# NomaDamas/AutoRAG-Research

Hardware: AMD Instinct MI355X
Metric: queries/sec (higher is better)
Workload: dtype f32

## Files before the change

autorag_research_amd/csrc/index.h:

```cpp
#pragma once
#include <climits>
#include <hip/hip_runtime.h>

#include <algorithm>
#include <cmath>
#include <cstdio>
#include <cstring>
#include <mutex>
#include <string>
#include <vector>

#include "dev_common.h"
#include "mi355dr.h"

namespace mi355 {
struct EventPair {
    hipEvent_t a, b;
    int big;
};
struct MultiVecStore;
struct Pending {
    bool active = false;
    hipEvent_t done = nullptr;
    int* status_host = nullptr;
// ... 30 lines not shown
    mi355::I8Group* grp8 = nullptr;
    int32_t* irr8_rows = nullptr;
    int* irr8_count = nullptr;
    int irr8_n = 0;

    bool qstate_ready = false;
    mi355::QueryState st{};
    float* qdev = nullptr;
    int32_t* cand_row = nullptr;
    float* cand_val = nullptr;
    int* qlist_dev = nullptr;
    int* status_or_dev = nullptr;
    int* status_host = nullptr;
    double* out_dist_dev = nullptr;
    int64_t* out_rows_dev = nullptr;
    unsigned long long* stat_dev = nullptr;
    int* prune_skip = nullptr;
    int prune_parity = 0;

    int path = 0;
    int screen_dtype = 0;
    int retry_level = 0;
    int i8_backoff = 0, i8_probation = 0;
    int i8_demoted_k = INT_MAX;
    double i8_min_budget = 0.25;
    float* retry_q[3] = {nullptr, nullptr, nullptr};
    double* retry_dist[3] = {nullptr, nullptr, nullptr};
    int64_t* retry_rows[3] = {nullptr, nullptr, nullptr};
    int* retry_map[3] = {nullptr, nullptr, nullptr};
    mi355::Pending pend[mi355::kPendingRing];
    mi355::Pending sub_pend[4];
    int64_t seq_next = 0, seq_done = 0;
    int k_now = 10;
    bool screening_now = false;
    int maxsim_coop = -1;
    int maxsim_persistent = 0;
    int maxsim_wg = -1;
    int maxsim_tighten = 1;
    int maxsim_aligned = 1;
    int maxsim_wg_min = 8;
    int maxsim_wg_pipe = 1;
    int maxsim_pack8 = -1;
    int maxsim_wg_bps = 4;
    int maxsim_pass_groups = 4;
    int maxsim_screen = 1;
    int64_t row_offset = 0;
    int round_a = 0;
    int screen_rq = 1;
    int screen_stream = 1;
    int prefilter16 = 0;
    int profile = 0;
    int starter = 1;
    int prune_companion = 1;
    int scan_dma = 1;
    int defer_round_b = 1;
    int chunk0_set = 0;
    int64_t chunk0_rows = 1024;
    int64_t chunk_growth = 3;
    int chunk_growth_set = 0;
    int64_t small_chunk_rows = 16384;
    int cap = mi355::kCandCap;
    int cap_set = 0;
    int prune_wide = 1;
    int screen_flush_sync = 1, screen_flush_lanes = 48, screen_flush_alone = 40;
    int wide_inflation_x10 = 100;
    int flush_mask_now = -1;
    int chunk_taper_x100 = 0;
    int64_t starter_rows_wide = 65536;

    int64_t s_screen_launches = 0, s_screen_ns = 0, s_screen_rows = 0, s_fallback_queries = 0, s_chunks = 0,
            s_passes = 0, s_candidates = 0, s_rescored = 0, s_starters = 0;
    int64_t s_big_launches = 0, s_big_ns = 0, s_big_rows = 0;
    int screen_rq_split_tests = 1;
    int64_t debug_park = 0;
    float* park_thr = nullptr;
    int screen_drift = 3;
    int* rq_progress = nullptr;
    int rq_epoch = 0;
    int64_t s_rq_launches = 0;
    int64_t s_retry_queries = 0;
    int64_t s_ms_screened = 0, s_ms_candidates = 0, s_ms_fallbacks = 0;
    int64_t s_ms_screen_ns = 0, s_ms_screen_launches = 0, s_ms_exact_ns = 0, s_ms_exact_launches = 0, s_ms_pack_ns = 0;
    int64_t s_ms_packed_launches = 0;
    int64_t s_ms_packed_blocks = 0;
    int64_t s_ms_packed_built = 0;
    int64_t s_ms_screen_cols = 0;
    hipEvent_t ms_ev[4] = {nullptr, nullptr, nullptr, nullptr};
    std::vector<mi355::EventPair> ev_pool, ev_pending;
    hipEvent_t t0 = nullptr, t1 = nullptr;

    void* comm = nullptr;
    int comm_rank = 0, comm_world = 0;
    mi355dr_allgather_fn comm_custom = nullptr;
    void* comm_custom_user = nullptr;
    int64_t* comm_packed[2] = {nullptr, nullptr};
    int64_t* comm_packed_all[2] = {nullptr, nullptr};
    hipStream_t comm_stream = nullptr;
    hipEvent_t comm_done[2] = {nullptr, nullptr};
    bool comm_done_armed[2] = {false, false};
    size_t comm_cap = 0;

    mi355::MultiVecStore* mv = nullptr;
};


namespace mi355 {
// ... 35 lines not shown
```

autorag_research_amd/csrc/k_select.h:

```cpp
#pragma once
#include "dev_common.h"

namespace mi355 {

struct PruneArgs {
    const float* rows;
    const float* nrm2;
    const float* q;
    QueryState st;
    int32_t* cand_row;
    float* cand_val;
    const int* qlist;
    unsigned long long* stat;
    int cap, d, k, metric;
    int exact;
    const uint8_t* flag8;
    float cscale;
    const uint16_t* shadow16;
    int dpad;
    int round_a;
    int* skip_list;
    int skip_parity;
    int thr_only;
    int one_wave_only;
    int defer_b;
};

__device__ __forceinline__ float unit_sim(int metric, double dist, float inv_qn) {
    return metric == 0 ? (float)(1.0 - dist) : (float)(-dist) * inv_qn;
}
__device__ __forceinline__ float screen_threshold(int metric, double dist_k, float E, float nq) {
    if (metric == 0) return float_below((float)((1.0 - dist_k) - (double)E));
    const double u = -dist_k / sqrt((double)nq);
    return float_below((float)(u - fabs(u) * 4e-6 - (double)E));
}

constexpr int kPruneSmallThreads = 64, kPruneSmallSort = 1024;
constexpr int kPruneBigThreads = 256, kPruneBigSort = kSortMax;

__host__ __device__ inline size_t prune_qs_floats(int d) { return ((size_t)d + 3) / 4 * 4 + 16; }
__host__ __device__ inline size_t prune_lds_bytes(int d, int threads, int sortmax, int dpad16) {
    size_t x = (size_t)(threads / kWave) * kStageFloats * sizeof(float);
    size_t lf = (size_t)sortmax * sizeof(float);
    if (lf > x) x = lf;
    return (size_t)sortmax * 8 + (size_t)sortmax * 4 + x + (size_t)sortmax * 4 + prune_qs_floats(d) * 4 + (size_t)dpad16 * 4;
}

template <int PER, int T, bool ROWS = false>
__device__ __forceinline__ void load_candidate_keys(uint32_t (&key)[PER], const float* __restrict__ cval,
                                                    const int32_t* __restrict__ crow, const uint8_t* __restrict__ flag8,
                                                    int n_new, int tid, int32_t* rows_out = nullptr) {
    float v[PER];
    int32_t r[PER];
    const int last = n_new - 1;
#pragma unroll
    for (int j = 0; j < PER; ++j) {
        v[j] = 0.0f;
        r[j] = 0;
        if (j * T >= n_new) continue;
        v[j] = cval[min(j * T + tid, last)];
        if (ROWS) r[j] = crow[min(j * T + tid, last)];
    }
    uint8_t f[PER];
#pragma unroll
    for (int j = 0; j < PER; ++j) f[j] = 0;
    if (flag8 != nullptr) {
        if (!ROWS) {
#pragma unroll
            for (int j = 0; j < PER; ++j) {
                if (j * T >= n_new) continue;
                r[j] = crow[min(j * T + tid, last)];
            }
        }
#pragma unroll
        for (int j = 0; j < PER; ++j) {
            if (j * T >= n_new) continue;
            f[j] = flag8[r[j]];
        }
    }
// ... 3 lines not shown
        if (j * T + tid < n_new) {
            if (v[j] != v[j]) kk = 0xFFFFFFFFu;
            else if (!f[j]) kk = f32_order_key(v[j]);
        }
        key[j] = kk;
        if (ROWS) rows_out[j] = r[j];
    }
}

template <int THREADS, int SORT>
__device__ __forceinline__ void prune_body(const PruneArgs& a, char* smem);

template <int THREADS, int SORT>
__global__ __launch_bounds__(THREADS) void k_prune(PruneArgs a) {
    extern __shared__ __attribute__((aligned(16))) char smem[];
    const bool list_mode = a.skip_list != nullptr && a.qlist == nullptr;
    const int tid = threadIdx.x;
    const int lane = tid & 63, wave = tid >> 6;
    int q = a.qlist ? a.qlist[blockIdx.x] : blockIdx.x;
    if (SORT == kPruneBigSort && list_mode) {
        if (blockIdx.x == 0 && tid == 0) a.skip_list[a.skip_parity ^ 1] = 0;
        const int n_left = a.skip_list[a.skip_parity];
        for (int i = blockIdx.x; i < n_left; i += gridDim.x) {
            PruneArgs b = a;
            b.skip_list = nullptr;
            b.qlist = a.skip_list + 2 + a.skip_parity * kQBlockMax + i - 0;
            b.qlist -= blockIdx.x;
            prune_body<THREADS, SORT>(b, smem);
            __syncthreads();
        }
        return;
    }
    prune_body<THREADS, SORT>(a, smem);
}

template <int THREADS, int SORT>
__device__ __forceinline__ void prune_body(const PruneArgs& a, char* smem) {
    constexpr int kWaves = THREADS / kWave;
    uint64_t* SK = (uint64_t*)smem;
    int32_t* SR = (int32_t*)(smem + (size_t)SORT * 8);
    char* X = smem + (size_t)SORT * 12;
    constexpr size_t xa = (size_t)kWaves * kStageFloats * sizeof(float), xb = (size_t)SORT * sizeof(float);
    constexpr size_t xbytes = xa > xb ? xa : xb;
    float* Lf = (float*)X;
    float* tiles = (float*)X;
    int32_t* R = (int32_t*)(X + xbytes);
    float* qs = (float*)(X + xbytes + (size_t)SORT * 4);
    int& s_cnt = *(int*)(X + xbytes + (size_t)SORT * 4 + (prune_qs_floats(a.d) - 16) * 4);
    float* q16 = qs + prune_qs_floats(a.d);
    const bool list_mode = a.skip_list != nullptr && a.qlist == nullptr;
    const int q = a.qlist ? a.qlist[blockIdx.x] : blockIdx.x;
    const int tid = threadIdx.x;
    const int lane = tid & 63, wave = tid >> 6;
    const int raw_cnt = a.st.cnt[q];
    const int n_best = a.st.best_n[q];
    if (raw_cnt == 0) return;
    if (a.exact && SORT < kPruneBigSort) return;
    auto leave_for_general = [&]() {
        if (a.one_wave_only) {
            if (tid == 0) {
                a.st.status[q] |= kStOverflow;
                a.st.cnt[q] = 0;
            }
            return;
        }
        if (list_mode && tid == 0) {
            const int i = atomicAdd(&a.skip_list[a.skip_parity], 1);
            a.skip_list[2 + a.skip_parity * kQBlockMax + i] = q;
        }
    };
    if (raw_cnt > a.cap) {
        if (SORT < kPruneBigSort) {
            leave_for_general();
            return;
        }
        if (tid == 0) {
            a.st.status[q] |= kStOverflow;
            a.st.cnt[q] = 0;
        }
        return;
    }
    if (n_best + raw_cnt > SORT) {
        if (SORT < kPruneBigSort) {
            leave_for_general();
            return;
        }
        if (tid == 0) {
            a.st.status[q] |= kStOverflow;
            a.st.cnt[q] = 0;
        }
        return;
    }
    const int n_new = raw_cnt;
    const int32_t* crow = a.cand_row + (int64_t)q * a.cap;
    const float* cval = a.cand_val + (int64_t)q * a.cap;
    uint64_t* bkey = a.st.best_key + (int64_t)q * kKMax;
    int32_t* brow = a.st.best_row + (int64_t)q * kKMax;
    const float nq = a.st.qn[q];
    const float inv_qn = 1.0f / sqrtf(nq);
    const float E = a.st.E[q];
    if (tid == 0) {
        a.stat[2 * q] += (unsigned long long)(n_new - a.st.carry[q]);
        a.st.carry[q] = 0;
    }

    int n_res;
    int n_base = n_best;
    bool kept_loaded = false;
    if constexpr (THREADS == kWave) {
        if (!a.exact) {
            float* tile = tiles;
            uint32_t key[kSelPerLane];
            unsigned in_a = 0;
            load_candidate_keys<kSelPerLane, kWave>(key, cval, crow, a.flag8, n_new, lane);
            for (int k = lane; k < a.d; k += kWave) qs[k] = a.q[(int64_t)q * a.d + k];
            if (a.shadow16 != nullptr)
                for (int k = lane; k < a.dpad; k += kWave) q16[k] = bf16_bits_to_f32(a.st.qhat[(int64_t)q * a.dpad + k]);
            const int n_cand = wave_count_ge(key, 1u, n_new);
            auto rescore_list = [&](int n, int dst) __attribute__((always_inline)) {
                for (int base = 0; base < n; base += kWave) {
                    const int e = base + lane;
                    const bool live = e < n;
                    const int32_t row = live ? crow[R[e]] : -1;
                    const float* rp = live ? a.rows + (int64_t)row * a.d : nullptr;
                    const float acc = staged_dot(tile, rp, qs, a.d, lane);
                    if (live) {
                        SK[dst + e] = dist_to_key(distance_from(a.metric, acc, nq, a.nrm2[row]));
                        SR[dst + e] = row;
                    }
                }
            };
            auto compact = [&](uint32_t x, int room, bool mark) -> int {
                int n = 0;
#pragma unroll
                for (int j = 0; j < kSelPerLane; ++j) {
                    if (j * kWave >= n_new) break;
                    const bool want = key[j] >= x && key[j] != 0 && !((in_a >> j) & 1u);
                    const unsigned long long bal = __builtin_amdgcn_ballot_w64(want);
                    const int pos = n + (int)__builtin_amdgcn_mbcnt_hi((unsigned)(bal >> 32),
                                                                       __builtin_amdgcn_mbcnt_lo((unsigned)bal, 0));
                    if (want && pos < room) {
                        R[pos] = j * kWave + lane;
                        if (mark) in_a |= 1u << j;
// ... 103 lines not shown
                    const int e = j * kWave + lane;
                    uint32_t kk = 0;
                    if (e < n_tot) kk = SK[e] == kKeyNaN ? 1u : f32_order_key(sim_of_dist(a.metric, key_to_dist(SK[e])));
                    sk[j] = kk;
                }
                const uint32_t xs = wave_nth_largest(sk, a.k, n_tot);
                n_sel = 0;
#pragma unroll
                for (int j = 0; j < kSelPerLane; ++j) {
                    if (j * kWave >= n_tot) break;
                    const bool want = sk[j] >= xs && sk[j] != 0;
                    const unsigned long long bal = __builtin_amdgcn_ballot_w64(want);
                    const int pos = n_sel + (int)__builtin_amdgcn_mbcnt_hi((unsigned)(bal >> 32),
                                                                           __builtin_amdgcn_mbcnt_lo((unsigned)bal, 0));
                    if (want) {
                        K2[pos] = SK[j * kWave + lane];
                        R2[pos] = SR[j * kWave + lane];
                    }
                    n_sel += __builtin_popcountll(bal);
                }
            } else {
                for (int i = lane; i < n_tot; i += kWave) {
                    K2[i] = SK[i];
                    R2[i] = SR[i];
                }
            }
            const int np = next_pow2(max(n_sel, 1));
            for (int i = n_sel + lane; i < np; i += kWave) {
                K2[i] = kKeyNaN;
                R2[i] = 0x7FFFFFFF;
            }
            __syncthreads();
            bitonic_asc_key_row(K2, R2, np);
            const int n_keep = min(a.k, n_sel);
            if (!a.thr_only)
                for (int i = lane; i < n_keep; i += kWave) {
                    bkey[i] = K2[i];
                    brow[i] = R2[i];
                }
            if (lane == 0) {
                if (!a.thr_only) a.st.best_n[q] = n_keep;
                a.st.cnt[q] = carried;
                a.st.carry[q] = carried;
                if (n_keep >= a.k) {
                    const uint64_t wk = K2[a.k - 1];
                    if (!a.thr_only) {
                        a.st.thr_key[q] = wk;
                        a.st.thr_row[q] = R2[a.k - 1];
                    }
                    if (wk != kKeyNaN && !(a.st.status[q] & kStIrregular))
                        a.st.thr[q] = screen_threshold(a.metric, key_to_dist(wk), E, nq);
                }
            }
            return;
        }
    }
    if (!a.exact) {
        const int nLp = next_pow2(n_new);
        for (int i = tid; i < nLp; i += THREADS) {
            float v = -__builtin_inff();
            if (i < n_new) {
                v = cval[i];
                if (v != v) v = __builtin_inff();
                else if (a.flag8 && a.flag8[crow[i]]) v = -__builtin_inff();
            }
            Lf[i] = v;
            R[i] = i;
        }
        if (tid == 0) s_cnt = 0;
        __syncthreads();
        bitonic_desc_f32_i32(Lf, R, nLp);
        for (int i = tid; i < nLp; i += THREADS)
            if (Lf[i] > -__builtin_inff() && (i + 1 == nLp || !(Lf[i + 1] > -__builtin_inff()))) s_cnt = i + 1;
        for (int k = tid; k < a.d; k += THREADS) qs[k] = a.q[(int64_t)q * a.d + k];
        __syncthreads();
        const int n_cand = s_cnt;
        __syncthreads();
        float* tile = tiles + wave * kStageFloats;
        auto rescore = [&](int e0, int e1, int dst) {
            for (int base = e0; base < e1; base += THREADS) {
                const int e = base + wave * kWave + lane;
                const bool live = e < e1;
                const int32_t row = live ? crow[R[e]] : -1;
                const float* rp = live ? a.rows + (int64_t)row * a.d : nullptr;
                float acc = 0.0f;
                if (base + wave * kWave < e1) acc = staged_dot(tile, rp, qs, a.d, lane);
                if (live) {
                    const double dist = distance_from(a.metric, acc, nq, a.nrm2[row]);
                    SK[dst + (e - e0)] = dist_to_key(dist);
                    SR[dst + (e - e0)] = row;
                }
            }
        };
        const int nA = min(n_cand, min(THREADS, max(32, 2 * a.k)));
        rescore(0, nA, n_best);
        int n_pass = nA;
        if (n_cand > nA) {
            for (int i = tid; i < n_best; i += THREADS) {
                SK[i] = bkey[i];
                SR[i] = brow[i];
            }
            kept_loaded = true;
            const int n1 = n_best + nA;
            const int np1 = next_pow2(n1);
            for (int i = n1 + tid; i < np1; i += THREADS) {
                SK[i] = kKeyNaN;
// ... 12 lines not shown
            }
            if (tid == 0) s_cnt = nA;
            __syncthreads();
            for (int i = nA + tid; i < n_cand; i += THREADS) {
                const float v = cval[R[i]];
                if (!(v < cut)) atomicMax(&s_cnt, i + 1);
            }
            __syncthreads();
            n_pass = s_cnt;
            rescore(nA, n_pass, n_base);
            n_res = n_pass - nA;
        } else {
            n_res = nA;
        }
        if (tid == 0) a.stat[2 * q + 1] += (unsigned long long)n_pass;
    } else {
        n_res = n_new;
        for (int i = tid; i < n_new; i += THREADS) {
            const int32_t row = crow[i];
            const double dist = distance_from(a.metric, cval[i], nq, a.nrm2[row]);
            SK[n_best + i] = dist_to_key(dist);
            SR[n_best + i] = row;
        }
    }
    if (!kept_loaded)
        for (int i = tid; i < n_best; i += THREADS) {
            SK[i] = bkey[i];
            SR[i] = brow[i];
        }
    const int n_tot = n_base + n_res;
    const int np = next_pow2(n_tot);
    for (int i = n_tot + tid; i < np; i += THREADS) {
        SK[i] = kKeyNaN;
        SR[i] = 0x7FFFFFFF;
    }
    __syncthreads();
    bitonic_asc_key_row(SK, SR, np);
    const int n_keep = min(a.k, n_tot);
    for (int i = tid; i < n_keep; i += THREADS) {
        bkey[i] = SK[i];
        brow[i] = SR[i];
    }
    if (tid == 0) {
        a.st.best_n[q] = n_keep;
        a.st.cnt[q] = 0;
        if (n_keep >= a.k) {
            const uint64_t wk = SK[a.k - 1];
            a.st.thr_key[q] = wk;
            a.st.thr_row[q] = SR[a.k - 1];
            if (!a.exact && wk != kKeyNaN && !(a.st.status[q] & kStIrregular))
                a.st.thr[q] = screen_threshold(a.metric, key_to_dist(wk), E, nq);
        }
    }
}

__global__ __launch_bounds__(64) void k_emit_irregular(const int32_t* __restrict__ irr_rows, int irr_n, QueryState st,
                                                        int32_t* cand_row, float* cand_val, int cap, int skip_below) {
    const int q = blockIdx.x;
    if (st.status[q] & kStIrregular) return;
    for (int i = threadIdx.x; i < irr_n; i += blockDim.x) {
        if (irr_rows[i] < skip_below) continue;
        const int slot = atomicAdd(&st.cnt[q], 1);
        if (slot < cap) {
            cand_row[(int64_t)q * cap + slot] = irr_rows[i];
            cand_val[(int64_t)q * cap + slot] = __builtin_nanf("");
        }
    }
}

__global__ __launch_bounds__(64) void k_finalize(QueryState st, int k, int64_t row_offset, double* out_dist,
                                                  int64_t* out_rows, int* status_or) {
    const int q = blockIdx.x;
    const int n = st.best_n[q];
    for (int s = threadIdx.x; s < k; s += blockDim.x) {
        if (s < n) {
            out_dist[(int64_t)q * k + s] = key_to_dist(st.best_key[(int64_t)q * kKMax + s]);
            out_rows[(int64_t)q * k + s] = (int64_t)st.best_row[(int64_t)q * kKMax + s] + row_offset;
        } else {
            out_dist[(int64_t)q * k + s] = __longlong_as_double(0x7FF8000000000000ll);
            out_rows[(int64_t)q * k + s] = -1;
        }
    }
    if (threadIdx.x == 0 && st.status[q] != 0) atomicOr(status_or, st.status[q]);
}

__global__ __launch_bounds__(256) void k_merge_topk(const double* __restrict__ dist_all,
                                                     const int64_t* __restrict__ rows_all, int64_t rank_stride, int world,
                                                     int B, int k, double* out_dist, int64_t* out_rows) {
    extern __shared__ __attribute__((aligned(16))) char smem[];
    uint64_t* SK = (uint64_t*)smem;
    const int np_ = next_pow2(world * k);
    int32_t* SI = (int32_t*)(smem + (size_t)np_ * 8);
    const int q = blockIdx.x;
    const int n = world * k;
    const int np = next_pow2(n);
    for (int i = threadIdx.x; i < np; i += blockDim.x) {
        if (i < n) {
            const int w = i / k, s = i % k;
            const int64_t src = (int64_t)w * rank_stride + (int64_t)q * k + s;
            const int64_t r = rows_all[src];
            SK[i] = r < 0 ? kKeyNaN : dist_to_key(dist_all[src]);
            SI[i] = r < 0 ? 0x7FFFFFFF : i;
        } else {
            SK[i] = kKeyNaN;
            SI[i] = 0x7FFFFFFF;
        }
// ... 51 lines not shown
```

autorag_research_amd/csrc/mi355dr.hip:

```cpp
#include "index.h"
#include "k_prep.h"
#include "k_scan.h"
#include "k_screen.h"
#include "k_screen256c.h"
#include "k_screen_rq.h"

#define MI355_RQ_FORMS(X) X(1) X(2) X(3) X(4) X(5) X(6)
inline bool screen_rq_has(int ksteps) { return ksteps >= 1 && ksteps <= 6; }
#include "k_screen_stream.h"
#include "k_select.h"
#include "k_prune_wide.h"

using namespace mi355;

namespace {
std::mutex g_err_mu;
std::string g_err;
}

namespace mi355 {
int fail(mi355dr_index* idx, int code, const std::string& msg) {
    if (idx) idx->err = msg;
    else {
        std::lock_guard<std::mutex> g(g_err_mu);
// ... 142 lines not shown

EventPair take_events(mi355dr_index* idx) {
    if (!idx->ev_pool.empty()) {
        EventPair p = idx->ev_pool.back();
        idx->ev_pool.pop_back();
        return p;
    }
    EventPair p{};
    (void)hipEventCreate(&p.a);
    (void)hipEventCreate(&p.b);
    return p;
}

void drain_events(mi355dr_index* idx) {
    std::vector<EventPair> keep;
    for (auto& p : idx->ev_pending) {
        if (hipEventQuery(p.b) == hipErrorNotReady) {
            keep.push_back(p);
            continue;
        }
        float ms = 0.f;
        if (hipEventElapsedTime(&ms, p.a, p.b) == hipSuccess) {
            idx->s_screen_ns += (int64_t)(ms * 1e6);
            if (p.big) idx->s_big_ns += (int64_t)(ms * 1e6);
        }
        idx->ev_pool.push_back(p);
    }
    idx->ev_pending.swap(keep);
}

constexpr double kInflationBf16 = 5.0, kInflationI8 = 16.0;
constexpr double kSmallBlockBudget = 1.6;
constexpr double kInflationI8Wide = 10.0, kInflationBf16Wide = 4.0;
inline bool wide_ok(const mi355dr_index* idx, int k) { return idx->prune_wide && k >= kWideKMin && k <= kWideKMax; }
inline bool wide_now(const mi355dr_index* idx) { return idx->screening_now && wide_ok(idx, idx->k_now); }
inline int cap_now(const mi355dr_index* idx) { return !idx->cap_set && wide_now(idx) ? kCandCapWide : idx->cap; }
inline double growth_budget(const mi355dr_index* idx, int k, bool i8) {
    if (wide_ok(idx, k) && idx->path != MI355DR_PATH_SCAN) {
        const int room = std::min(kWideEntries, idx->cap_set ? idx->cap : kCandCapWide);
        return 0.75 * room / ((double)k * (i8 ? idx->wide_inflation_x10 / 10.0 : kInflationBf16Wide)) - 1.0;
    }
    const int room = k < kPruneSmallSort / 2 ? kPruneSmallSort - k : idx->cap;
    return 0.6 * std::min(room, idx->cap) / ((double)k * (i8 ? kInflationI8 : kInflationBf16));
}

inline bool i8_available(const mi355dr_index* idx) { return idx->irr8_n <= kIrrCap; }
inline bool use_i8(const mi355dr_index* idx) {
    if (idx->retry_level > 0) return false;
    if (idx->screen_dtype == MI355DR_SCREEN_I8) return true;
    return idx->screen_dtype == MI355DR_SCREEN_AUTO && i8_available(idx) && idx->k_now < idx->i8_demoted_k &&
           growth_budget(idx, idx->k_now, true) >= idx->i8_min_budget;
}

int launch_prune(mi355dr_index* idx, hipStream_t s, int nblocks, const int* qlist, int k, int exact, bool thr_only = false,
                 bool one_wave_only = false, bool defer_b = false) {
    PruneArgs pa{};
    pa.thr_only = thr_only ? 1 : 0;
    pa.one_wave_only = one_wave_only ? 1 : 0;
    pa.defer_b = defer_b && idx->defer_round_b ? 1 : 0;
    pa.rows = idx->rows;
    pa.nrm2 = idx->nrm2;
    pa.q = idx->qdev;
    pa.st = idx->st;
    pa.cand_row = idx->cand_row;
    pa.cand_val = idx->cand_val;
    pa.qlist = qlist;
    pa.stat = idx->stat_dev;
    pa.cap = cap_now(idx);
    pa.d = idx->dim;
    pa.k = k;
    pa.metric = idx->metric;
    pa.exact = exact;
    pa.flag8 = (use_i8(idx) && idx->irr8_n > 0) ? idx->flag8 : nullptr;
    pa.cscale = idx->metric == MI355DR_METRIC_IP ? idx->cmax : 1.0f;
    pa.shadow16 = (use_i8(idx) && idx->metric == 0 && !exact && idx->prefilter16) ? idx->shadow : nullptr;
    pa.dpad = idx->dpad;
    pa.round_a = idx->round_a;
    if (!exact && wide_now(idx)) {
        pa.shadow16 = nullptr;
        hipLaunchKernelGGL((k_prune_wide<2, 32>), dim3(nblocks), dim3(2 * kWave), prune_wide_lds_bytes(idx->dim, 2), s, pa);
        HIPCHECK(idx, hipGetLastError());
        return MI355DR_OK;
    }
    if (pa.cap > kCandCap) return fail(idx, MI355DR_E_INTERNAL, "general-form prune on a list stride above kCandCap");
    const bool list_mode = qlist == nullptr;
    pa.skip_list = list_mode ? idx->prune_skip : nullptr;
    pa.skip_parity = list_mode ? (idx->prune_parity ^= 1) : 0;
    hipLaunchKernelGGL((k_prune<kPruneSmallThreads, kPruneSmallSort>), dim3(nblocks), dim3(kPruneSmallThreads),
                       prune_lds_bytes(idx->dim, kPruneSmallThreads, kPruneSmallSort, pa.shadow16 ? idx->dpad : 0), s, pa);
    HIPCHECK(idx, hipGetLastError());
    if (one_wave_only) return MI355DR_OK;
    hipLaunchKernelGGL((k_prune<kPruneBigThreads, kPruneBigSort>), dim3(list_mode ? std::min(nblocks, 64) : nblocks),
                       dim3(kPruneBigThreads), prune_lds_bytes(idx->dim, kPruneBigThreads, kPruneBigSort, 0), s, pa);
    HIPCHECK(idx, hipGetLastError());
    return MI355DR_OK;
}

int launch_prep(mi355dr_index* idx, hipStream_t s, int B, int Bpad, int metric, int cnt0 = 0) {
    hipLaunchKernelGGL(k_prep_queries, dim3(Bpad), dim3(64), (size_t)idx->dim * sizeof(float), s, idx->qdev, B, idx->dim,
                       idx->dpad, metric, idx->st, idx->dpad8, use_i8(idx) ? 1 : 0, idx->bf16_ec, idx->status_or_dev,
                       idx->prune_skip, cnt0, idx->metric == MI355DR_METRIC_IP ? idx->cmax : 1.0f);
    idx->prune_parity = 0;
    HIPCHECK(idx, hipGetLastError());
    return MI355DR_OK;
}

inline int screen_tile(int B) { return B > kTileN ? kT2 : kTileM; }

constexpr int kRetryLevels = 2;

__global__ void k_set_counts(int* cnt, int n, int v) {
    const int i = blockIdx.x * blockDim.x + threadIdx.x;
    if (i < n) cnt[i] = v;
}

int launch_screen(mi355dr_index* idx, hipStream_t s, int B, int64_t r0, int64_t r_end, int cap, int emit_mode) {
    const bool emit_all = emit_mode != 0;
    const int tile = (emit_all || r_end - r0 <= idx->small_chunk_rows) ? kTileM : screen_tile(B);
    const bool i8 = use_i8(idx);
    ScreenArgs2 sa{};
    sa.status = idx->st.status;
    sa.shadow = i8 ? (const void*)idx->shadow8 : (const void*)idx->shadow;
    sa.qhat = i8 ? (const void*)idx->st.qhat8 : (const void*)idx->st.qhat;
    sa.thr = idx->st.thr;
    sa.sc = idx->st.sc;
    sa.kq = idx->st.kq;
    sa.grp = idx->grp8;
    sa.flag8 = idx->flag8;
    sa.cnt = idx->st.cnt;
    sa.cand_row = idx->cand_row;
    sa.cand_val = idx->cand_val;
    sa.row_bytes = i8 ? idx->dpad8 : idx->dpad * 2;
    sa.ksteps = sa.row_bytes / kRowB;
    sa.cap = cap;
    sa.ct0 = (int)(r0 / tile);
    sa.n_ctiles = (int)(round_up(r_end, tile) / tile) - sa.ct0;
    sa.n_qtiles = (int)(round_up(B, tile) / tile);
    sa.row_end = r_end;
// ... 74 lines not shown
    if (idx->starter && (k <= kStarterKMax || wide) && idx->retry_level == 0 && idx->chunk0_set == 0 && n >= 4 * 1024 &&
        starter_slabs <= cap && starter_slabs >= k) {
        p.sample = starter_rows;
        seen = p.sample;
    } else {
        const int64_t c0 = std::min<int64_t>(n, round_up(std::max<int64_t>(tile, std::min<int64_t>(idx->chunk0_rows, cap)), tile));
        p.emit_all_first = c0 <= cap;
        p.ends.push_back(c0);
        seen = c0;
        if (c0 >= n) return p;
    }
    const double rmax = 1.0 + growth;
    const double span = (double)n / (double)seen;
    int steps = std::max(1, (int)std::ceil(std::log(span) / std::log(rmax) - 0.15));
    const double r = std::pow(span, 1.0 / steps);
    double taper = std::max(1.0, (idx->chunk_taper_x100 > 0 ? idx->chunk_taper_x100 : (wide ? 120 : 100)) / 100.0);
    if (steps > 1 && taper > 1.0) {
        const double room = std::max(1.0, rmax * 1.25 / r);
        taper = std::min(taper, std::pow(room, 2.0 / (steps - 1)));
    } else {
        taper = 1.0;
    }
    double pos = (double)seen;
    int64_t prev = p.sample > 0 ? 0 : seen;
    for (int i = 1; i <= steps; ++i) {
        pos *= r * std::pow(taper, (steps - 1) / 2.0 - (i - 1));
        int64_t end = i == steps ? n : std::min<int64_t>(n, round_up((int64_t)pos, tile));
        if (tile == kT2 && end < n) {
            const int n_qtiles = (int)(round_up(B, kT2) / kT2);
            const int64_t round_rows = (int64_t)8 * (32 / n_qtiles) * kT2;
            const int64_t len = end - prev;
            if (len >= 2 * round_rows) end = std::min<int64_t>(n, prev + (len + round_rows / 2) / round_rows * round_rows);
        }
        if (end <= prev) continue;
        p.ends.push_back(end);
        prev = end;
        if (end >= n) break;
    }
    if (p.ends.empty() || p.ends.back() < n) p.ends.push_back(n);
    return p;
}

inline int starter_count(const PassPlan& p) { return (int)((p.sample + kSlabRows - 1) / kSlabRows); }

PassPlan make_plan(const mi355dr_index* idx, int B, int k) {
    double growth = std::max(0.25, std::min((double)idx->chunk_growth, growth_budget(idx, k, use_i8(idx))));
    if (B <= 64 && idx->retry_level == 0 && idx->chunk_growth_set == 0)
        growth = std::max(growth, std::min(8.0, growth_budget(idx, k, use_i8(idx)) * kSmallBlockBudget));
    if (idx->retry_level == 1) growth = std::max(0.25, growth * 0.5);
    if (idx->retry_level >= 2) growth = 0.25;
    return plan_pass(idx, B, k, growth);
}

int run_screen(mi355dr_index* idx, hipStream_t s, int B, int k, const PassPlan& plan) {
    int64_t kept_all_below = 0;
    const bool i8 = use_i8(idx);
    const int side_n = i8 ? idx->irr8_n : idx->irr_n;
    constexpr int kSideMerge = 32;
    bool side_done = false;
    const bool lean = plan.sample > 0 && idx->prune_companion == 0;
    auto timed = [&](bool big, int64_t rows, auto&& launch) -> int {
        EventPair ev{};
        if (idx->profile) {
            ev = take_events(idx);
            HIPCHECK(idx, hipEventRecord(ev.a, s));
        }
        CHECK(launch());
        if (idx->profile) {
            HIPCHECK(idx, hipEventRecord(ev.b, s));
            ev.big = big ? 1 : 0;
            idx->ev_pending.push_back(ev);
        }
        idx->s_screen_launches++;
        idx->s_screen_rows += rows;
        if (big) {
            idx->s_big_launches++;
            idx->s_big_rows += rows;
        }
        return MI355DR_OK;
    };
    if (plan.sample > 0) {
        CHECK(timed(false, plan.sample, [&] { return launch_screen(idx, s, B, 0, plan.sample, cap_now(idx), kEmitSlabMax); }));
        CHECK(launch_prune(idx, s, B, nullptr, k, 0, true, true));
        idx->s_starters++;
    }
    int64_t done = 0;
    for (size_t ci = 0; ci < plan.ends.size(); ++ci) {
        const int64_t end = plan.ends[ci];
        const bool emit_all = ci == 0 && plan.emit_all_first;
        if (emit_all) kept_all_below = end;
        const bool big = !emit_all && end - done > idx->small_chunk_rows && screen_tile(B) == kT2;
        {
            const int64_t seen = ci == 0 ? (plan.sample > 0 ? plan.sample : end) : done;
            const double lanes = 8.0 * k * 4096.0 / (double)std::max<int64_t>(seen, 1);
            int period = 1;
            while (period < 64 && period * 2 * lanes <= idx->screen_flush_lanes) period *= 2;
            idx->flush_mask_now = idx->screen_flush_sync ? period - 1 : -1;
        }
        CHECK(timed(big, end - done, [&] { return launch_screen(idx, s, B, done, end, cap_now(idx), emit_all ? kEmitAll : 0); }));
        idx->s_chunks++;
        if (end >= idx->n && side_n > 0 && side_n <= kSideMerge) {
            hipLaunchKernelGGL(k_emit_irregular, dim3(B), dim3(64), 0, s, i8 ? idx->irr8_rows : idx->irr_rows, side_n, idx->st,
                               idx->cand_row, idx->cand_val, cap_now(idx), (int)kept_all_below);
            HIPCHECK(idx, hipGetLastError());
            side_done = true;
        }
        const bool last = end >= idx->n && (side_n == 0 || side_done);
        CHECK(launch_prune(idx, s, B, nullptr, k, 0, false, lean, !last));
        done = end;
    }
    if (side_n > 0 && !side_done) {
        hipLaunchKernelGGL(k_emit_irregular, dim3(B), dim3(64), 0, s, i8 ? idx->irr8_rows : idx->irr_rows, side_n, idx->st,
                           idx->cand_row, idx->cand_val, cap_now(idx), (int)kept_all_below);
        HIPCHECK(idx, hipGetLastError());
        CHECK(launch_prune(idx, s, B, nullptr, k, 0, false, lean));
    }
    idx->s_passes++;
    return MI355DR_OK;
}

__global__ void k_reset_queries(QueryState st, const int* qlist, int nq) {
    const int i = blockIdx.x * blockDim.x + threadIdx.x;
    if (i >= nq) return;
    const int q = qlist[i];
    st.cnt[q] = 0;
    st.carry[q] = 0;
    st.best_n[q] = 0;
    st.thr_key[q] = kKeyNaN;
    st.thr_row[q] = 0x7FFFFFFF;
    st.status[q] &= ~kStOverflow;
}

int scan_range(mi355dr_index* idx, hipStream_t s, int off, int nq, int k, int64_t r0, int64_t r1) {
    ScanArgs sa{};
    sa.rows = idx->rows;
    sa.nrm2 = idx->nrm2;
    sa.q = idx->qdev;
    sa.st = idx->st;
    sa.cand_row = idx->cand_row;
    sa.cand_val = idx->cand_val;
    sa.qlist = idx->qlist_dev + off;
    sa.nq = nq;
    sa.cap = cap_now(idx);
    sa.d = idx->dim;
    sa.metric = idx->metric;
    sa.row0 = r0;
    sa.row1 = r1;
    const int64_t grid = (r1 - r0 + kScanThreads - 1) / kScanThreads;
    if (idx->dim % kScan32PieceCols == 0 && idx->scan_dma)
        hipLaunchKernelGGL(k_scan32, dim3((unsigned)grid), dim3(kScanThreads), kScan32Lds, s, sa, idx->n);
    else
        hipLaunchKernelGGL(k_scan, dim3((unsigned)grid), dim3(kScanThreads), scan_lds_bytes(idx->dim, nq), s, sa);
    HIPCHECK(idx, hipGetLastError());
    return launch_prune(idx, s, nq, idx->qlist_dev + off, k, 1);
}

int run_scan(mi355dr_index* idx, hipStream_t s, const std::vector<int>& qs, int k) {
    if (qs.empty()) return MI355DR_OK;
    HIPCHECK(idx, hipMemcpyAsync(idx->qlist_dev, qs.data(), qs.size() * sizeof(int), hipMemcpyHostToDevice, s));
    const int nq_all = (int)qs.size();
    hipLaunchKernelGGL(k_reset_queries, dim3((nq_all + 255) / 256), dim3(256), 0, s, idx->st, idx->qlist_dev, nq_all);
    HIPCHECK(idx, hipGetLastError());
    const int per = kScanQ;
    for (int off = 0; off < nq_all; off += per) {
        const int nq = std::min(per, nq_all - off);
        int64_t done = 0;
        const int cap = cap_now(idx);
        int64_t chunk = std::min<int64_t>(idx->chunk0_rows, cap);
// ... 15 lines not shown
                    for (int q : redo)
                        HIPCHECK(idx, hipMemcpyAsync(idx->st.status + q, idx->status_host + q, sizeof(int),
                                                     hipMemcpyHostToDevice, s));
                    for (int64_t p = done; p < end; p += cap)
                        CHECK(scan_range(idx, s, roff, (int)redo.size(), k, p, std::min<int64_t>(end, p + cap)));
                }
            }
            done = end;
            chunk = std::max<int64_t>(chunk, done * (idx->chunk_growth_set ? idx->chunk_growth : 63));
        }
    }
    idx->s_fallback_queries += nq_all;
    return MI355DR_OK;
}

__global__ void k_gather_queries(const float* src, const int* map, int d, float* dst) {
    const int j = blockIdx.x;
    for (int c = threadIdx.x; c < d; c += blockDim.x) dst[(int64_t)j * d + c] = src[(int64_t)map[j] * d + c];
}
__global__ void k_scatter_results(const double* sd, const int64_t* sr, const int* map, int k, double* od, int64_t* orow) {
    const int j = blockIdx.x;
    for (int i = threadIdx.x; i < k; i += blockDim.x) {
        od[(int64_t)map[j] * k + i] = sd[(int64_t)j * k + i];
        orow[(int64_t)map[j] * k + i] = sr[(int64_t)j * k + i];
    }
}

int pending_alloc(mi355dr_index* idx, Pending& p) {
    if (!p.status_host) HIPCHECK(idx, hipHostMalloc(&p.status_host, (kQBlockMax + 1) * sizeof(int)));
    if (!p.done) HIPCHECK(idx, hipEventCreateWithFlags(&p.done, hipEventDisableTiming));
    return MI355DR_OK;
}

int enqueue_block(mi355dr_index* idx, hipStream_t s, const float* q_dev, int B, int k, double* out_dist_dev,
                  int64_t* out_rows_dev, Pending& p) {
    CHECK(ensure_qstate(idx));
    CHECK(pending_alloc(idx, p));
    idx->k_now = k;
    if (idx->retry_level == 0 && idx->screen_dtype == MI355DR_SCREEN_AUTO && k >= idx->i8_demoted_k && --idx->i8_probation <= 0)
        idx->i8_demoted_k = INT_MAX;
    const int Bpad = (int)round_up(B, screen_tile(B));
    if (idx->screen_dtype == MI355DR_SCREEN_I8 && !i8_available(idx) && idx->path != MI355DR_PATH_SCAN)
        return fail(idx, MI355DR_E_UNSUPPORTED, "int8 screen unavailable: too many rows outside the residual limit");
    const bool screen_possible = use_i8(idx) ? i8_available(idx) : idx->irr_n <= kIrrCap;
    const bool use_screen = idx->n > 0 && screen_possible && idx->path != MI355DR_PATH_SCAN;
    idx->screening_now = use_screen;
    if (idx->path == MI355DR_PATH_SCREEN && !screen_possible && idx->n > 0)
        return fail(idx, MI355DR_E_UNSUPPORTED, "screen path unavailable (metric or too many irregular rows)");
    if (q_dev != idx->qdev)
        HIPCHECK(idx, hipMemcpyAsync(idx->qdev, q_dev, (size_t)B * idx->dim * sizeof(float), hipMemcpyDeviceToDevice, s));
    PassPlan plan;
    if (use_screen) plan = make_plan(idx, B, k);
    CHECK(launch_prep(idx, s, B, Bpad, idx->metric, starter_count(plan)));
    if (idx->n > 0) {
        if (use_screen) {
            CHECK(run_screen(idx, s, B, k, plan));
        } else {
            std::vector<int> all(B);
            for (int i = 0; i < B; ++i) all[i] = i;
            CHECK(run_scan(idx, s, all, k));
        }
    }
    hipLaunchKernelGGL(k_finalize, dim3(B), dim3(64), 0, s, idx->st, k, idx->row_offset, out_dist_dev, out_rows_dev,
                       idx->status_or_dev);
    HIPCHECK(idx, hipGetLastError());
    HIPCHECK(idx, hipMemcpyAsync(p.status_host, idx->st.status, (size_t)(kQBlockMax + 1) * sizeof(int), hipMemcpyDeviceToHost, s));
    HIPCHECK(idx, hipEventRecord(p.done, s));
    p.active = true;
    p.stream = s;
    p.q_dev = q_dev;
    p.B = B;
    p.k = k;
    p.out_dist = out_dist_dev;
    p.out_rows = out_rows_dev;
    p.used_screen = use_screen;
    p.was_i8 = use_screen && use_i8(idx);
    p.level = idx->retry_level;
    return MI355DR_OK;
}

int search_block(mi355dr_index* idx, hipStream_t s, const float* q_dev, int B, int k, double* out_dist_dev,
                 int64_t* out_rows_dev);

int complete_block(mi355dr_index* idx, Pending& p) {
    if (!p.active) return MI355DR_OK;
    p.active = false;
    HIPCHECK(idx, hipEventSynchronize(p.done));
    drain_events(idx);
    if (!p.used_screen) {
        for (int i = 0; i < p.B; ++i)
            if (p.status_host[i] & kStOverflow)
                return fail(idx, MI355DR_E_INTERNAL, "exact scan: query " + std::to_string(i) + " lost a candidate chunk");
        return MI355DR_OK;
    }
    if (p.status_host[kQBlockMax] == 0) return MI355DR_OK;
    hipStream_t s = p.stream;
    const int B = p.B, k = p.k, level = p.level;
    std::vector<int> sub;
    int n_todo = 0;
    {
        std::vector<int> retry;
        for (int i = 0; i < B; ++i) {
            const int st = p.status_host[i];
            if (st == 0) continue;
            if (level < kRetryLevels && !(st & kStIrregular)) retry.push_back(i);
            else sub.push_back(i);
        }
        n_todo = (int)sub.size();
        sub.insert(sub.end(), retry.begin(), retry.end());
    }
    const int n_sub = (int)sub.size(), n_retry = n_sub - n_todo;
    if (n_sub == 0) return MI355DR_OK;
    if (!idx->retry_q[level]) {
        HIPCHECK(idx, hipMalloc(&idx->retry_q[level], (size_t)kQBlockMax * idx->dim * sizeof(float)));
        HIPCHECK(idx, hipMalloc(&idx->retry_dist[level], (size_t)kQBlockMax * kKMax * sizeof(double)));
        HIPCHECK(idx, hipMalloc(&idx->retry_rows[level], (size_t)kQBlockMax * kKMax * sizeof(int64_t)));
        HIPCHECK(idx, hipMalloc(&idx->retry_map[level], (size_t)kQBlockMax * sizeof(int)));
    }
// ... 366 lines not shown
    }
    const std::string k(key);
    if (k == "path") {
        if (value < 0 || value > 2) return fail(idx, MI355DR_E_INVALID, "path must be 0,1,2");
        idx->path = (int)value;
    } else if (k == "screen_dtype") {
        if (value < 0 || value > 2) return fail(idx, MI355DR_E_INVALID, "screen_dtype must be 0,1,2");
        idx->screen_dtype = (int)value;
        idx->i8_demoted_k = INT_MAX;
        idx->i8_backoff = idx->i8_probation = 0;
    } else if (k == "i8_min_budget_x100") {
        if (value < 1 || value > 1000) return fail(idx, MI355DR_E_INVALID, "i8_min_budget_x100 must be in 1..1000");
        idx->i8_min_budget = (double)value / 100.0;
    } else if (k == "maxsim_screen") {
        idx->maxsim_screen = value != 0;
    } else if (k == "maxsim_coop") {
        if (value < -1 || value > 1) return fail(idx, MI355DR_E_INVALID, "maxsim_coop must be -1 (by document length), 0 or 1");
        idx->maxsim_coop = (int)value;
    } else if (k == "maxsim_persistent") {
        idx->maxsim_persistent = value != 0;
    } else if (k == "maxsim_wg") {
        if (value < -1 || value > 2) return fail(idx, MI355DR_E_INVALID, "maxsim_wg must be -1 (by document length), 0, 1 or 2");
        idx->maxsim_wg = (int)value;
    } else if (k == "maxsim_tighten") {
        idx->maxsim_tighten = value != 0;
    } else if (k == "maxsim_aligned") {
        idx->maxsim_aligned = value != 0;
    } else if (k == "maxsim_wg_min") {
        if (value < 8 || value > 9) return fail(idx, MI355DR_E_INVALID, "maxsim_wg_min must be 8 or 9");
        idx->maxsim_wg_min = (int)value;
    } else if (k == "maxsim_wg_pipe") {
        idx->maxsim_wg_pipe = value != 0;
    } else if (k == "maxsim_pack8") {
        if (value < -1 || value > 1) return fail(idx, MI355DR_E_INVALID, "maxsim_pack8 must be -1 (when it pays), 0 or 1");
        idx->maxsim_pack8 = (int)value;
    } else if (k == "maxsim_wg_bps") {
        if (value != 2 && value != 4) return fail(idx, MI355DR_E_INVALID, "maxsim_wg_bps must be 2 or 4");
        idx->maxsim_wg_bps = (int)value;
    } else if (k == "maxsim_pass_groups") {
        if (value < 1 || value > 4) return fail(idx, MI355DR_E_INVALID, "maxsim_pass_groups must be in 1..4");
        idx->maxsim_pass_groups = (int)value;
    } else if (k == "row_offset") {
        idx->row_offset = value;
    } else if (k == "profile") {
        idx->profile = value != 0;
    } else if (k == "chunk0_rows") {
        if (value < 1) return fail(idx, MI355DR_E_INVALID, "chunk0_rows must be >= 1");
        idx->chunk0_rows = value;
        idx->chunk0_set = 1;
    } else if (k == "starter") {
        idx->starter = value != 0;
    } else if (k == "prune_companion") {
        idx->prune_companion = value != 0;
    } else if (k == "scan_dma") {
        idx->scan_dma = value != 0;
    } else if (k == "defer_round_b") {
        idx->defer_round_b = value != 0;
    } else if (k == "chunk_growth") {
        if (value < 1) return fail(idx, MI355DR_E_INVALID, "chunk_growth must be >= 1");
        idx->chunk_growth = value;
        idx->chunk_growth_set = 1;
    } else if (k == "screen_stream") {
        idx->screen_stream = value != 0;
    } else if (k == "screen_rq") {
        idx->screen_rq = value != 0;
    } else if (k == "debug_park_thresholds") {
        idx->debug_park = value;
    } else if (k == "screen_rq_split_tests") {
        idx->screen_rq_split_tests = value != 0;
    } else if (k == "screen_drift") {
        if (value < 0 || value > 1024) return fail(idx, MI355DR_E_INVALID, "screen_drift: 0 ... 1024 tiles");
        idx->screen_drift = (int)value;
    } else if (k == "small_chunk_rows") {
        if (value < 0) return fail(idx, MI355DR_E_INVALID, "small_chunk_rows must be >= 0");
        idx->small_chunk_rows = value;
    } else if (k == "round_a") {
        if (value < 0 || value > 64) return fail(idx, MI355DR_E_INVALID, "round_a must be in [0,64]");
        idx->round_a = (int)value;
    } else if (k == "prefilter16") {
        idx->prefilter16 = value != 0;
    } else if (k == "cand_cap") {
        if (value < 16 || value > kCandCap) return fail(idx, MI355DR_E_INVALID, "cand_cap must be in [16,2048]");
        idx->cap = (int)value;
        idx->cap_set = 1;
    } else if (k == "prune_wide") {
        idx->prune_wide = value != 0;
    } else if (k == "screen_flush_sync") {
        idx->screen_flush_sync = value != 0;
    } else if (k == "screen_flush_lanes") {
        if (value < 1 || value > 64) return fail(idx, MI355DR_E_INVALID, "screen_flush_lanes must be in [1, 64]");
        idx->screen_flush_lanes = (int)value;
    } else if (k == "screen_flush_alone") {
        if (value < 8 || value > 60) return fail(idx, MI355DR_E_INVALID, "screen_flush_alone must be in [8, 60]");
        idx->screen_flush_alone = (int)value;
    } else if (k == "wide_inflation_x10") {
        if (value < 20 || value > 400) return fail(idx, MI355DR_E_INVALID, "wide_inflation_x10 must be in [20, 400]");
        idx->wide_inflation_x10 = (int)value;
    } else if (k == "chunk_taper_x100") {
        if (value != 0 && (value < 100 || value > 300)) return fail(idx, MI355DR_E_INVALID, "chunk_taper_x100 must be 0 (auto) or in [100, 300]");
        idx->chunk_taper_x100 = (int)value;
    } else if (k == "starter_rows_wide") {
        if (value < 4096 || value > 262144) return fail(idx, MI355DR_E_INVALID, "starter_rows_wide must be in [4096, 262144]");
        idx->starter_rows_wide = value;
    } else {
        return fail(idx, MI355DR_E_INVALID, "unknown option: " + k);
    }
// ... 234 lines not shown
```

Before: 163,800.

## Fuse irregular-row emission and finalize into the last prune launch

When the final screen pass runs the single-wave prune, the irregular side rows are now appended to the candidate list inside the prune kernel. The prune kernel then writes the final distances and rows directly, so the separate k_emit_irregular and k_finalize launches are skipped. This removes up to two small kernel launches per search block, which matters at high query rates. It adds complexity to the prune kernel. Early-exit and overflow paths must now write outputs or status consistently, and the fused path is refused for wide and list modes.

```diff
diff --git a/autorag_research_amd/csrc/index.h b/autorag_research_amd/csrc/index.h
--- a/autorag_research_amd/csrc/index.h
+++ b/autorag_research_amd/csrc/index.h
@@ -106,6 +106,7 @@
     int profile = 0;
     int starter = 1;
     int prune_companion = 1;
+    int fused_tail = 1;
     int scan_dma = 1;
     int defer_round_b = 1;
     int chunk0_set = 0;
diff --git a/autorag_research_amd/csrc/k_select.h b/autorag_research_amd/csrc/k_select.h
--- a/autorag_research_amd/csrc/k_select.h
+++ b/autorag_research_amd/csrc/k_select.h
@@ -24,7 +24,31 @@
     int thr_only;
     int one_wave_only;
     int defer_b;
+    const int32_t* side_rows;
+    int side_n, side_skip;
+    int finalize;
+    int64_t row_offset;
+    double* out_dist;
+    int64_t* out_rows;
+    int* status_or;
 };
+
+template <int THREADS>
+__device__ __forceinline__ void finalize_query(const PruneArgs& a, int q, const uint64_t* K, const int32_t* R, int n, int tid) {
+    for (int s = tid; s < a.k; s += THREADS) {
+        if (s < n) {
+            a.out_dist[(int64_t)q * a.k + s] = key_to_dist(K[s]);
+            a.out_rows[(int64_t)q * a.k + s] = (int64_t)R[s] + a.row_offset;
+        } else {
+            a.out_dist[(int64_t)q * a.k + s] = __longlong_as_double(0x7FF8000000000000ll);
+            a.out_rows[(int64_t)q * a.k + s] = -1;
+        }
+    }
+    if (tid == 0) {
+        const int st = a.st.status[q];
+        if (st != 0) atomicOr(a.status_or, st);
+    }
+}
 
 __device__ __forceinline__ float unit_sim(int metric, double dist, float inv_qn) {
     return metric == 0 ? (float)(1.0 - dist) : (float)(-dist) * inv_qn;
@@ -134,16 +158,42 @@
     const int q = a.qlist ? a.qlist[blockIdx.x] : blockIdx.x;
     const int tid = threadIdx.x;
     const int lane = tid & 63, wave = tid >> 6;
-    const int raw_cnt = a.st.cnt[q];
+    int raw_cnt = a.st.cnt[q];
     const int n_best = a.st.best_n[q];
-    if (raw_cnt == 0) return;
+    if constexpr (THREADS == kWave) {
+        if (a.side_n > 0 && !(a.st.status[q] & kStIrregular)) {
+            const int32_t row = lane < a.side_n ? a.side_rows[lane] : -1;
+            const bool mine = row >= a.side_skip && lane < a.side_n;
+            const unsigned long long bal = __builtin_amdgcn_ballot_w64(mine);
+            const int slot = raw_cnt + (int)__builtin_amdgcn_mbcnt_hi((unsigned)(bal >> 32),
+                                                                      __builtin_amdgcn_mbcnt_lo((unsigned)bal, 0));
+            if (mine && slot < a.cap) {
+                a.cand_row[(int64_t)q * a.cap + slot] = row;
+                a.cand_val[(int64_t)q * a.cap + slot] = __builtin_nanf("");
+            }
+            raw_cnt += __builtin_popcountll(bal);
+            if (lane == 0) a.st.cnt[q] = raw_cnt;
+            asm volatile("s_waitcnt vmcnt(0)" ::: "memory");
+            wave_sync();
+        }
+    }
+    auto flag_overflow = [&]() {
+        if (tid == 0) {
+            const int st = a.st.status[q] | kStOverflow;
+            a.st.status[q] = st;
+            a.st.cnt[q] = 0;
+            if (a.finalize) atomicOr(a.status_or, st);
+        }
+    };
+    if (raw_cnt == 0) {
+        if (a.finalize)
+            finalize_query<THREADS>(a, q, a.st.best_key + (int64_t)q * kKMax, a.st.best_row + (int64_t)q * kKMax, n_best, tid);
+        return;
+    }
     if (a.exact && SORT < kPruneBigSort) return;
     auto leave_for_general = [&]() {
         if (a.one_wave_only) {
-            if (tid == 0) {
-                a.st.status[q] |= kStOverflow;
-                a.st.cnt[q] = 0;
-            }
+            flag_overflow();
             return;
         }
         if (list_mode && tid == 0) {
@@ -156,10 +206,7 @@
             leave_for_general();
             return;
         }
-        if (tid == 0) {
-            a.st.status[q] |= kStOverflow;
-            a.st.cnt[q] = 0;
-        }
+        flag_overflow();
         return;
     }
     if (n_best + raw_cnt > SORT) {
@@ -167,10 +214,7 @@
             leave_for_general();
             return;
         }
-        if (tid == 0) {
-            a.st.status[q] |= kStOverflow;
-            a.st.cnt[q] = 0;
-        }
+        flag_overflow();
         return;
     }
     const int n_new = raw_cnt;
@@ -380,6 +424,7 @@
                         a.st.thr[q] = screen_threshold(a.metric, key_to_dist(wk), E, nq);
                 }
             }
+            if (a.finalize) finalize_query<THREADS>(a, q, K2, R2, n_keep, lane);
             return;
         }
     }
@@ -498,6 +543,7 @@
                 a.st.thr[q] = screen_threshold(a.metric, key_to_dist(wk), E, nq);
         }
     }
+    if (a.finalize) finalize_query<THREADS>(a, q, SK, SR, n_keep, tid);
 }
 
 __global__ __launch_bounds__(64) void k_emit_irregular(const int32_t* __restrict__ irr_rows, int irr_n, QueryState st,
diff --git a/autorag_research_amd/csrc/mi355dr.hip b/autorag_research_amd/csrc/mi355dr.hip
--- a/autorag_research_amd/csrc/mi355dr.hip
+++ b/autorag_research_amd/csrc/mi355dr.hip
@@ -218,9 +218,26 @@
            growth_budget(idx, idx->k_now, true) >= idx->i8_min_budget;
 }
 
+struct PruneTail {
+    const int32_t* side_rows = nullptr;
+    int side_n = 0, side_skip = 0;
+    double* out_dist = nullptr;
+    int64_t* out_rows = nullptr;
+};
+
 int launch_prune(mi355dr_index* idx, hipStream_t s, int nblocks, const int* qlist, int k, int exact, bool thr_only = false,
-                 bool one_wave_only = false, bool defer_b = false) {
+                 bool one_wave_only = false, bool defer_b = false, const PruneTail* tail = nullptr) {
     PruneArgs pa{};
+    if (tail) {
+        pa.side_rows = tail->side_rows;
+        pa.side_n = tail->side_n;
+        pa.side_skip = tail->side_skip;
+        pa.finalize = 1;
+        pa.row_offset = idx->row_offset;
+        pa.out_dist = tail->out_dist;
+        pa.out_rows = tail->out_rows;
+        pa.status_or = idx->status_or_dev;
+    }
     pa.thr_only = thr_only ? 1 : 0;
     pa.one_wave_only = one_wave_only ? 1 : 0;
     pa.defer_b = defer_b && idx->defer_round_b ? 1 : 0;
@@ -243,6 +260,7 @@
     pa.dpad = idx->dpad;
     pa.round_a = idx->round_a;
     if (!exact && wide_now(idx)) {
+        if (tail) return fail(idx, MI355DR_E_INTERNAL, "two-wave prune asked for a fused tail");
         pa.shadow16 = nullptr;
         hipLaunchKernelGGL((k_prune_wide<2, 32>), dim3(nblocks), dim3(2 * kWave), prune_wide_lds_bytes(idx->dim, 2), s, pa);
         HIPCHECK(idx, hipGetLastError());
@@ -250,6 +268,7 @@
     }
     if (pa.cap > kCandCap) return fail(idx, MI355DR_E_INTERNAL, "general-form prune on a list stride above kCandCap");
     const bool list_mode = qlist == nullptr;
+    if (tail && !list_mode) return fail(idx, MI355DR_E_INTERNAL, "fused tail on a query list");
     pa.skip_list = list_mode ? idx->prune_skip : nullptr;
     pa.skip_parity = list_mode ? (idx->prune_parity ^= 1) : 0;
     hipLaunchKernelGGL((k_prune<kPruneSmallThreads, kPruneSmallSort>), dim3(nblocks), dim3(kPruneSmallThreads),
@@ -430,13 +449,19 @@
     return plan_pass(idx, B, k, growth);
 }
 
-int run_screen(mi355dr_index* idx, hipStream_t s, int B, int k, const PassPlan& plan) {
+int run_screen(mi355dr_index* idx, hipStream_t s, int B, int k, const PassPlan& plan, double* out_dist, int64_t* out_rows,
+               bool* finalized) {
     int64_t kept_all_below = 0;
     const bool i8 = use_i8(idx);
     const int side_n = i8 ? idx->irr8_n : idx->irr_n;
     constexpr int kSideMerge = 32;
     bool side_done = false;
     const bool lean = plan.sample > 0 && idx->prune_companion == 0;
+    const bool fuse = idx->fused_tail && !wide_now(idx);
+    PruneTail tail{};
+    tail.out_dist = out_dist;
+    tail.out_rows = out_rows;
+    *finalized = false;
     auto timed = [&](bool big, int64_t rows, auto&& launch) -> int {
         EventPair ev{};
         if (idx->profile) {
@@ -478,20 +503,28 @@
         CHECK(timed(big, end - done, [&] { return launch_screen(idx, s, B, done, end, cap_now(idx), emit_all ? kEmitAll : 0); }));
         idx->s_chunks++;
         if (end >= idx->n && side_n > 0 && side_n <= kSideMerge) {
-            hipLaunchKernelGGL(k_emit_irregular, dim3(B), dim3(64), 0, s, i8 ? idx->irr8_rows : idx->irr_rows, side_n, idx->st,
-                               idx->cand_row, idx->cand_val, cap_now(idx), (int)kept_all_below);
-            HIPCHECK(idx, hipGetLastError());
+            if (fuse) {
+                tail.side_rows = i8 ? idx->irr8_rows : idx->irr_rows;
+                tail.side_n = side_n;
+                tail.side_skip = (int)kept_all_below;
+            } else {
+                hipLaunchKernelGGL(k_emit_irregular, dim3(B), dim3(64), 0, s, i8 ? idx->irr8_rows : idx->irr_rows, side_n,
+                                   idx->st, idx->cand_row, idx->cand_val, cap_now(idx), (int)kept_all_below);
+                HIPCHECK(idx, hipGetLastError());
+            }
             side_done = true;
         }
         const bool last = end >= idx->n && (side_n == 0 || side_done);
-        CHECK(launch_prune(idx, s, B, nullptr, k, 0, false, lean, !last));
+        CHECK(launch_prune(idx, s, B, nullptr, k, 0, false, lean, !last, last && fuse ? &tail : nullptr));
+        if (last && fuse) *finalized = true;
         done = end;
     }
     if (side_n > 0 && !side_done) {
         hipLaunchKernelGGL(k_emit_irregular, dim3(B), dim3(64), 0, s, i8 ? idx->irr8_rows : idx->irr_rows, side_n, idx->st,
                            idx->cand_row, idx->cand_val, cap_now(idx), (int)kept_all_below);
         HIPCHECK(idx, hipGetLastError());
-        CHECK(launch_prune(idx, s, B, nullptr, k, 0, false, lean));
+        CHECK(launch_prune(idx, s, B, nullptr, k, 0, false, lean, false, fuse ? &tail : nullptr));
+        if (fuse) *finalized = true;
     }
     idx->s_passes++;
     return MI355DR_OK;
@@ -613,18 +646,21 @@
     PassPlan plan;
     if (use_screen) plan = make_plan(idx, B, k);
     CHECK(launch_prep(idx, s, B, Bpad, idx->metric, starter_count(plan)));
+    bool finalized = false;
     if (idx->n > 0) {
         if (use_screen) {
-            CHECK(run_screen(idx, s, B, k, plan));
+            CHECK(run_screen(idx, s, B, k, plan, out_dist_dev, out_rows_dev, &finalized));
         } else {
             std::vector<int> all(B);
             for (int i = 0; i < B; ++i) all[i] = i;
             CHECK(run_scan(idx, s, all, k));
         }
     }
-    hipLaunchKernelGGL(k_finalize, dim3(B), dim3(64), 0, s, idx->st, k, idx->row_offset, out_dist_dev, out_rows_dev,
-                       idx->status_or_dev);
-    HIPCHECK(idx, hipGetLastError());
+    if (!finalized) {
+        hipLaunchKernelGGL(k_finalize, dim3(B), dim3(64), 0, s, idx->st, k, idx->row_offset, out_dist_dev, out_rows_dev,
+                           idx->status_or_dev);
+        HIPCHECK(idx, hipGetLastError());
+    }
     HIPCHECK(idx, hipMemcpyAsync(p.status_host, idx->st.status, (size_t)(kQBlockMax + 1) * sizeof(int), hipMemcpyDeviceToHost, s));
     HIPCHECK(idx, hipEventRecord(p.done, s));
     p.active = true;
@@ -1097,6 +1133,9 @@
         idx->starter = value != 0;
     } else if (k == "prune_companion") {
         idx->prune_companion = value != 0;
+    } else if (k == "fused_tail") {
+        idx->fused_tail = value != 0;
+
     } else if (k == "scan_dma") {
         idx->scan_dma = value != 0;
     } else if (k == "defer_round_b") {
```

Result: no change. 163,900 (median of 2 runs) (+0.1%).
